# hsinnan75/MapCaller

Measured on AMD Instinct MI355X. Metric: reads/sec (150 bp PE vs GRCh38) at 1/2/4/8 MI355X; SAM CIGAR bit-exact, higher is better.
Workload: dtype u64/int32; 1 GPU; synthetic GRCh38-sized genome, 3100 Mbp (synthetic: GRCh38 is unavailable offline; repeat landscape in the detail record), 4000000 pairs x 150 bp PE per step per GPU (sub 0.005, ins 0.001, del 0.001 per base), -alg ksw2

## Files before the change

include/mcx.h:

```cpp
#ifndef MCX_H
#define MCX_H
#include <stdint.h>

#ifdef __cplusplus
extern "C" {
#endif

typedef struct mcx_index mcx_index;
typedef struct mcx_ctx mcx_ctx;

enum mcx_status {
    MCX_OK = 0,
    MCX_ERR_IO = -1,
    MCX_ERR_ARG = -2,
    MCX_ERR_DEVICE = -3,
    MCX_ERR_CAPACITY = -4,
    MCX_ERR_UNSUPPORTED = -5
};

const char *mcx_last_error(void);
int mcx_device_count(void);

#define MCX_INDEX_SAMPLED 0
#define MCX_INDEX_FULL 1
// ... 20 lines not shown
    int64_t max_batch_reads;
} mcx_opts;
void mcx_opts_default(mcx_opts *);

int mcx_ctx_create(const mcx_index *, const mcx_opts *, mcx_ctx **out);
typedef struct mcx_fit {
    int32_t pair_records_trimmed;
    int32_t batch_halvings;
    int32_t single_detail_set;
    int32_t pad;
    int64_t max_batch_reads;
    int64_t hbm_free_bytes;
    int64_t hbm_taken_bytes;
} mcx_fit;
int mcx_ctx_create_fit(mcx_index *, const mcx_opts *, int with_profile, int paired, int max_dup, int max_clip, mcx_ctx **out, uint32_t **planes, mcx_fit *fit);
void mcx_ctx_free(mcx_ctx *);

int mcx_bwt_search_batch(mcx_ctx *, const uint8_t *seqs, const uint32_t *seq_off, const int32_t *start, uint32_t n,
                         int32_t *len, int32_t *freq, uint64_t *loc);
int mcx_extend_batch(mcx_ctx *, int alg, const uint8_t *q, const uint32_t *q_off, const uint8_t *t,
                     const uint32_t *t_off, uint32_t n, uint8_t *ops, int32_t *ops_len, int32_t *score);
int mcx_extend_lanes(mcx_ctx *, int alg, int form, int strip, uint32_t blocks, const uint8_t *q, const uint32_t *q_off, const uint8_t *t,
                     const uint32_t *t_off, uint32_t n, uint8_t *ops, int32_t *ops_len, int32_t *score, void *summaries);

typedef struct mcx_aln {
    int64_t pos;
    int64_t mate_pos;
    int32_t chr;
    int32_t flag;
    int32_t mapq;
    int32_t tlen;
    int32_t nm, as, xs;
    int32_t n_cigar;
    int32_t fwd;
    int32_t has_mate;
    int32_t cigar_off;
    int32_t pad;
} mcx_aln;

typedef struct mcx_aln32 {
    uint32_t pos_lo, mate_lo;
    uint8_t pos_hi, mate_hi;
    uint8_t mapq;
    uint8_t bits;
    int32_t tlen;
    uint16_t flag;
// ... 140 lines not shown
```

mapcaller_amd/api.py:

```python
from __future__ import annotations

import ctypes as C
import os
from typing import List, Optional, Tuple

import numpy as np

_HERE = os.path.dirname(os.path.abspath(__file__))
LIB_PATH = os.environ.get("MCX_LIB") or os.path.join(_HERE, "libmcx.so")
CIGAR_STRIDE = 32
CIGAR_SLACK = 65536


def cigar_pool_words(n_reads):
    return n_reads * CIGAR_STRIDE + CIGAR_SLACK


def pack_reads(bases, lens=None):
    import torch
    n, rlen = bases.shape
    row_words = (rlen + 15) // 16
    lut = torch.zeros(256, dtype=torch.int64, device=bases.device)
    for i, ch in enumerate(b"ACGT"):
        lut[ch] = i
# ... 3 lines not shown
    b64 = bases.long()
    if lens is None:
        lens_t = torch.full((n,), rlen, dtype=torch.int64, device=bases.device)
    else:
        lens_t = lens.to(bases.device).long()
    inside = torch.arange(rlen, device=bases.device)[None, :] < lens_t[:, None]
    codes = lut[b64] * inside
    pad = row_words * 16 - rlen
    if pad:
        codes = torch.nn.functional.pad(codes, (0, pad))
    shifts = (30 - 2 * torch.arange(16, device=bases.device)).long()
    words = (codes.reshape(n, row_words, 16) << shifts).sum(-1)
    words = torch.where(words >= 2 ** 31, words - 2 ** 32, words).to(torch.int32)
    bad = (~known[b64]) & inside
    r, pos = torch.nonzero(bad, as_tuple=True)
    odd = (r << 32) | (pos << 8) | b64[r, pos]
    return (words.contiguous().cpu().pin_memory(), lens_t.to(torch.int32).cpu().pin_memory(), odd.cpu().pin_memory() if odd.numel() else torch.zeros(1, dtype=torch.int64).pin_memory(),
            int(odd.numel()), row_words)


SYMBOLS = [
    "mcx_last_error", "mcx_device_count", "mcx_pack_row", "mcx_host_cpus", "mcx_gz_inflate", "mcx_index_load", "mcx_index_build", "mcx_index_from_codes", "mcx_index_save", "mcx_index_free", "mcx_index_trim",
    "mcx_index_genome_size", "mcx_index_n_chr", "mcx_index_chr_name", "mcx_index_chr_len", "mcx_index_hbm_bytes",
    "mcx_opts_default", "mcx_ctx_create", "mcx_ctx_create_fit", "mcx_ctx_free", "mcx_bwt_search_batch", "mcx_extend_batch", "mcx_extend_lanes",
    "mcx_avg_init", "mcx_map_batch_dev", "mcx_map_batch", "mcx_cigar_words", "mcx_map_files", "mcx_map_files_ex", "mcx_file_opts_default",
    "mcx_profile_attach", "mcx_profile_settle", "mcx_profile_finalize", "mcx_profile_sparse", "mcx_planes_alloc", "mcx_planes_free", "mcx_planes_bytes",
    "mcx_vcf_defaults", "mcx_call_variants",
    "mcx_batch_begin", "mcx_batch_sums", "mcx_batch_replay", "mcx_batch_end", "mcx_avg_walk", "mcx_batch_totals", "mcx_batch_check", "mcx_avg_advance", "mcx_exchange_local", "mcx_exchange_local_free",
    "mcx_profile_sparse_shard", "mcx_batch_end_keys", "mcx_batch_accumulate",
    "mcx_stream_submit", "mcx_stream_submit_packed", "mcx_stream_map", "mcx_stream_collect", "mcx_stream_next", "mcx_stream_mapped",
    "mcx_stream_map32", "mcx_stream_mapped32",
    "mcx_ctx_set_multi", "mcx_multi_lines", "mcx_multi_copy", "mcx_stream_multi",
    "mcx_sam_format_dev", "mcx_sam_format", "mcx_sam_header",
]
COMM_LIB_PATH = os.path.join(_HERE, "libmcx_comm.so")
COMM_SYMBOLS = ["mcx_comm_init_all", "mcx_comm_unique_id", "mcx_comm_init_rank", "mcx_comm_free", "mcx_comm_rank", "mcx_comm_size",
                "mcx_profile_reduce", "mcx_comm_exchange", "mcx_comm_exchange_free"]


class McxError(RuntimeError):
    pass


class Opts(C.Structure):
    _fields_ = [("alg", C.c_int32), ("max_pos_diff", C.c_int32), ("max_mismatch_rate", C.c_float),
                ("max_read_len", C.c_int32), ("max_batch_reads", C.c_int64)]

# ... 184 lines not shown
    L.mcx_last_error.restype = C.c_char_p
    L.mcx_index_genome_size.restype = C.c_int64
    L.mcx_index_hbm_bytes.restype = C.c_int64
    L.mcx_index_chr_name.restype = C.c_char_p
    L.mcx_index_load.argtypes = [C.c_char_p, C.c_int, C.c_int, C.POINTER(C.c_void_p)]
    L.mcx_index_build.argtypes = [C.c_char_p, C.c_char_p, C.c_int]
    L.mcx_index_from_codes.argtypes = [C.c_void_p, C.c_int32, C.POINTER(C.c_int32), C.POINTER(C.c_char_p), C.c_int, C.c_int,
                                       C.POINTER(C.c_void_p), C.POINTER(C.c_double)]
    L.mcx_index_save.argtypes = [C.c_void_p, C.c_char_p]
    L.mcx_index_trim.argtypes = [C.c_void_p, C.c_int]
    for f in (L.mcx_index_free, L.mcx_ctx_free):
        f.argtypes = [C.c_void_p]
        f.restype = None
    for f in (L.mcx_index_genome_size, L.mcx_index_n_chr, L.mcx_index_hbm_bytes):
        f.argtypes = [C.c_void_p]
    L.mcx_index_chr_name.argtypes = [C.c_void_p, C.c_int32]
    L.mcx_index_chr_len.argtypes = [C.c_void_p, C.c_int32]
    L.mcx_opts_default.argtypes = [C.POINTER(Opts)]
    L.mcx_opts_default.restype = None
    L.mcx_ctx_create.argtypes = [C.c_void_p, C.POINTER(Opts), C.POINTER(C.c_void_p)]
    L.mcx_ctx_create_fit.argtypes = [C.c_void_p, C.POINTER(Opts), C.c_int, C.c_int, C.c_int, C.c_int, C.POINTER(C.c_void_p), C.POINTER(C.c_void_p), C.POINTER(Fit)]
    L.mcx_bwt_search_batch.argtypes = [C.c_void_p] + [C.c_void_p] * 3 + [C.c_uint32] + [C.c_void_p] * 3
    L.mcx_extend_batch.argtypes = [C.c_void_p, C.c_int] + [C.c_void_p] * 4 + [C.c_uint32] + [C.c_void_p] * 3
    L.mcx_extend_lanes.argtypes = [C.c_void_p, C.c_int, C.c_int, C.c_int, C.c_uint32] + [C.c_void_p] * 4 + [C.c_uint32] + [C.c_void_p] * 4
    L.mcx_avg_init.argtypes = [C.POINTER(C.c_int64)]
    L.mcx_avg_init.restype = None
    for f in (L.mcx_map_batch_dev, L.mcx_map_batch):
        f.argtypes = [C.c_void_p, C.c_void_p, C.c_void_p, C.c_uint32, C.c_int, C.POINTER(C.c_int64), C.c_void_p,
                      C.c_void_p, C.POINTER(Stats)]
    L.mcx_map_files.argtypes = [C.c_void_p, C.c_char_p, C.c_char_p, C.c_char_p, C.POINTER(Stats)]
    L.mcx_map_files_ex.argtypes = [C.c_void_p, C.c_char_p, C.c_char_p, C.POINTER(FileOpts), C.c_char_p, C.POINTER(Stats)]
    L.mcx_file_opts_default.argtypes = [C.POINTER(FileOpts)]
    L.mcx_file_opts_default.restype = None
    L.mcx_profile_attach.argtypes = [C.c_void_p, C.c_void_p, C.c_int, C.c_int]
    L.mcx_profile_settle.argtypes = [C.c_void_p]
    L.mcx_profile_finalize.argtypes = [C.c_void_p, C.c_void_p]
    L.mcx_profile_sparse.argtypes = [C.c_void_p, C.POINTER(C.POINTER(SparseRec)), C.POINTER(C.c_uint64)]
    L.mcx_profile_sparse_shard.argtypes = [C.c_void_p, C.POINTER(C.POINTER(SparseRec)), C.POINTER(C.c_uint64)]
    L.mcx_batch_begin.argtypes = [C.c_void_p, C.c_void_p, C.c_void_p, C.c_uint32, C.c_int, C.c_int32, C.c_int64, C.c_void_p, C.c_void_p, C.POINTER(Stats)]
    L.mcx_batch_sums.argtypes = [C.c_void_p, C.POINTER(C.c_uint32)] + [C.POINTER(C.POINTER(C.c_uint32))] * 3
    L.mcx_batch_replay.argtypes = [C.c_void_p, C.c_void_p, C.POINTER(C.c_uint32), C.POINTER(Stats)]
    L.mcx_batch_end.argtypes = [C.c_void_p, C.POINTER(Stats)]
    L.mcx_batch_end_keys.argtypes = [C.c_void_p, C.POINTER(Stats), C.POINTER(C.POINTER(C.c_uint64)), C.POINTER(C.c_uint64)]
    L.mcx_batch_accumulate.argtypes = [C.c_void_p, C.c_void_p, C.c_uint64, C.c_uint32, C.c_uint32]
    L.mcx_avg_walk.argtypes = [C.POINTER(C.c_int64), C.c_void_p, C.c_void_p, C.c_uint32, C.c_void_p]
    L.mcx_avg_walk.restype = None
# ... 394 lines not shown
        _check(lib().mcx_bwt_search_batch(self._h, buf.ctypes.data, off.ctypes.data, st.ctypes.data, n, ln.ctypes.data,
                                          fr.ctypes.data, loc.ctypes.data), "mcx_bwt_search_batch")
        return ln, fr, loc

    def extend(self, alg: str, qs: List[bytes], ts: List[bytes]):
        n = len(qs)
        qo = np.zeros(n + 1, dtype=np.uint32)
        to = np.zeros(n + 1, dtype=np.uint32)
        qo[1:] = np.cumsum([len(s) for s in qs])
        to[1:] = np.cumsum([len(s) for s in ts])
        qb = np.frombuffer(b"".join(qs), dtype=np.uint8).copy()
        tb = np.frombuffer(b"".join(ts), dtype=np.uint8).copy()
        ops = np.zeros(int(qo[-1]) + int(to[-1]) + 16, dtype=np.uint8)
        ol = np.zeros(n, dtype=np.int32)
        sc = np.zeros(n, dtype=np.int32)
        _check(lib().mcx_extend_batch(self._h, 0 if alg == "nw" else 1, qb.ctypes.data, qo.ctypes.data, tb.ctypes.data,
                                      to.ctypes.data, n, ops.ctypes.data, ol.ctypes.data, sc.ctypes.data), "mcx_extend_batch")
        out = []
        for i in range(n):
            b = int(qo[i]) + int(to[i])
            out.append(ops[b:b + int(ol[i])].tobytes().decode())
        return out, sc

    def extend_lanes(self, alg: str, form: int, strip: int, qs: List[bytes], ts: List[bytes], blocks: int = 0, summaries: bool = False):
        n = len(qs)
        qo = np.zeros(n + 1, dtype=np.uint32)
        to = np.zeros(n + 1, dtype=np.uint32)
        qo[1:] = np.cumsum([len(s) for s in qs])
        to[1:] = np.cumsum([len(s) for s in ts])
        qb = np.frombuffer(b"".join(qs) + b"\0", dtype=np.uint8).copy()
        tb = np.frombuffer(b"".join(ts) + b"\0", dtype=np.uint8).copy()
        ops = np.zeros(int(qo[-1]) + int(to[-1]) + 16, dtype=np.uint8)
        ol = np.zeros(n, dtype=np.int32)
        sc = np.zeros(n, dtype=np.int32)
        sm = np.zeros(n, dtype=DP_SUMMARY_DTYPE) if summaries else None
        _check(lib().mcx_extend_lanes(self._h, 0 if alg == "nw" else 1, form, strip, blocks, qb.ctypes.data, qo.ctypes.data, tb.ctypes.data,
                                      to.ctypes.data, n, ops.ctypes.data, ol.ctypes.data, sc.ctypes.data, sm.ctypes.data if summaries else None),
               "mcx_extend_lanes")
        out = []
        for i in range(n):
            b = int(qo[i]) + int(to[i])
            out.append(ops[b:b + int(ol[i])].tobytes().decode())
        return out, ol, sc, sm

    def close(self):
        if self._h:
# ... 85 lines not shown
```

mapcaller_amd/csrc/mcx_ctx.h:

```cpp
#ifndef MCX_CTX_H
#define MCX_CTX_H
#include <hip/hip_runtime.h>
#include <algorithm>
#include <atomic>
#include <chrono>
#include <cmath>
#include <cstdio>
#include <cstdlib>
#include <cstring>
#include <string>
#include <type_traits>
#include <vector>

#include "../../include/mcx.h"
#include "mcx_dp.h"
#include "mcx_dp_lane2.h"
#include "mcx_simple.h"
#include "mcx_profile.h"
#include "mcx_internal.h"

using namespace mcx;

#define HIP_TRY(expr)                                                                                  \
    do {                                                                                               \
// ... 170 lines not shown
            uint32_t *h_index = nullptr, *h_cig = nullptr; mcx_aln32 *h_recs = nullptr; uint32_t h_rec_cap = 0, h_word_cap = 0;
        } mx;
    } slot[3];
    const Slot *collected = nullptr;
    hipStream_t h2d_stream = nullptr, d2h_stream = nullptr;
    uint64_t stream_seq = 0, stream_bytes_in = 0, stream_bytes_out = 0;
    void *d_scan_tmp = nullptr; size_t scan_tmp_bytes = 0;
    void *files_state = nullptr; void (*files_drop)(void *) = nullptr;
    void *sam_state = nullptr; void (*sam_drop)(void *) = nullptr;
    uint8_t *d_bases = nullptr; uint32_t *d_off = nullptr; AlnRec *d_recs = nullptr; uint32_t *d_cig = nullptr;
    struct Multi {
        bool on = false, ready = false;
        uint32_t rec_cap = 0, word_cap = 0;
        AlnRec *d_pool = nullptr; uint32_t *d_pool_cig = nullptr; uint32_t *d_cnt = nullptr; uint4 *d_ref = nullptr;
        uint32_t *d_counts = nullptr;
        uint32_t *d_index = nullptr, *d_windex = nullptr;
        AlnRec *d_out = nullptr; uint32_t *d_out_cig = nullptr; uint32_t out_cap = 0, out_wcap = 0;
        void *d_tmp = nullptr; size_t tmp_bytes = 0;
        uint32_t n_reads = 0, n_recs = 0, n_words = 0;
    } mx;
};

int reserve_tier0(mcx_ctx *c, int paired, uint64_t n_reads);
void pack_reads(const ReadBatch &rb, int paired, int wpad, int tpr, uint32_t *out, uint32_t *any_n, uint8_t *odd_flag, hipStream_t s);
int launch_dp(const Knobs &kn, const PassRes &R, const Ctx &cx, const JobSinks &sinks, const ReadBatch &rb, const PairSel &sel, int rlen_max);
uint64_t lane_short_words(int which);
uint64_t lane_stride_words(bool nw, int rows, int strips);
int profile_keys(mcx_ctx *c);
int profile_queue(mcx_ctx *c);
int profile_collect(mcx_ctx *c);
int archive_append(mcx_ctx *c, mcx_ctx::Archive &a, const SparseRec *d_src, uint64_t n, hipStream_t on = nullptr);
int profile_foreign(mcx_ctx *c, const uint64_t *h_all, uint64_t n_all);
int sort_reserve(mcx_ctx *c, uint64_t n);
int profile_accumulate(mcx_ctx *c, const uint64_t *h_all, uint64_t n_all, uint32_t slot_stride, uint32_t own_slot);

#endif
```

mapcaller_amd/csrc/mcx_pipeline.hip:

```cpp
#include "mcx_ctx.h"
#include <hipcub/hipcub.hpp>

static thread_local std::string g_err;
static int fail(int code, const std::string &msg) { g_err = msg; return code; }
int mcx_set_error(int code, const std::string &msg) { return fail(code, msg); }
extern "C" const char *mcx_last_error(void) { return g_err.c_str(); }
extern "C" int mcx_device_count(void)
{
    int n = 0;
    if (hipGetDeviceCount(&n) != hipSuccess) return 0;
    return n;
}

struct EndsLds { int64_t pos[kLdsEnds]; int32_t chr[kLdsEnds]; };

static __device__ __forceinline__ void stage_ends(IndexView &ix, EndsLds &l)
{
    if (ix.n_ends <= kLdsEnds) {
        for (int i = threadIdx.x; i < ix.n_ends; i += blockDim.x) { l.pos[i] = ix.end_pos[i]; l.chr[i] = ix.end_chr[i]; }
        __syncthreads();
        ix.end_pos = l.pos; ix.end_chr = l.chr;
    }
}

// ... 4 lines not shown
        uint32_t r = pair * nr + s;
        rd[s].ascii = rb.bases + rb.off[r];
        rd[s].rlen = (int32_t)(rb.off[r + 1] - rb.off[r]);
        rd[s].flipped = (cx.pm.paired && s == 1) ? 1 : 0;
        rd[s].codes = (cx.packed && !(cx.read_ext[r] >> 31)) ? cx.packed + (uint64_t)r * cx.wpad : nullptr;
#ifdef MCX_DEBUG_NO_CODES
        rd[s].codes = nullptr;
#endif
    }
}

struct SeedOut {
    uint2 *tasks;
    uint32_t *n_tasks;
    uint32_t task_cap;
    uint32_t *read_ext;
    uint32_t *read_blocks;
    const uint32_t *packed;
    int wpad;
    uint32_t *queue;
    const uint8_t *src_state; Layout src_lay; Caps src_caps;
};

static __device__ __forceinline__ U4 load16_unaligned(const uint8_t *p)
{
    const uintptr_t a = (uintptr_t)p;
    const U4 *q = (const U4 *)(a & ~(uintptr_t)15);
    const U4 lo = q[0];
    const unsigned sh = (unsigned)(a & 15);
    if (sh == 0) return lo;
    const U4 hi = q[1];
    const unsigned qd = sh >> 2, b = sh & 3;
    uint32_t s0, s1, s2, s3, s4;
    switch (qd) {
    case 0: s0 = lo.x; s1 = lo.y; s2 = lo.z; s3 = lo.w; s4 = hi.x; break;
    case 1: s0 = lo.y; s1 = lo.z; s2 = lo.w; s3 = hi.x; s4 = hi.y; break;
    case 2: s0 = lo.z; s1 = lo.w; s2 = hi.x; s3 = hi.y; s4 = hi.z; break;
    default: s0 = lo.w; s1 = hi.x; s2 = hi.y; s3 = hi.z; s4 = hi.w; break;
    }
    U4 r;
    r.x = __builtin_amdgcn_alignbyte(s1, s0, b); r.y = __builtin_amdgcn_alignbyte(s2, s1, b);
    r.z = __builtin_amdgcn_alignbyte(s3, s2, b); r.w = __builtin_amdgcn_alignbyte(s4, s3, b);
    return r;
}

static __device__ __forceinline__ void pack4(uint32_t w, bool comp, uint32_t &codes, uint32_t &flags, uint32_t &lower)
{
    const uint32_t c = w & 0xDFDFDFDFu;
    auto zero_bytes = [](uint32_t t) { return ~(((t & 0x7F7F7F7Fu) + 0x7F7F7F7Fu) | t | 0x7F7F7F7Fu); };
    const uint32_t member = (zero_bytes(c ^ 0x41414141u) | zero_bytes(c ^ 0x43434343u) | zero_bytes(c ^ 0x47474747u) | zero_bytes(c ^ 0x54545454u)) >> 7;
    const uint32_t h = (c >> 1) & 0x03030303u;
    uint32_t code = h ^ ((h >> 1) & 0x01010101u);
    if (comp) code ^= 0x03030303u;
    code &= member * 3u;
    const uint32_t y = __builtin_bswap32(code), n = __builtin_bswap32(member ^ 0x01010101u);
    codes = (y | (y >> 6) | (y >> 12) | (y >> 18)) & 0xFFu;
    flags = (n | (n >> 7) | (n >> 14) | (n >> 21)) & 0xFu;
    const uint32_t l = __builtin_bswap32((w >> 5) & 0x01010101u);
    lower = (l | (l >> 7) | (l >> 14) | (l >> 21)) & 0xFu;
}

static __device__ __forceinline__ void pack16(const ReadRef &rd, int i0, uint32_t &codes, uint32_t &flags, uint32_t &odd)
{
    const int rlen = rd.rlen;
    int n = rlen - i0; if (n > 16) n = 16;
    codes = 0; flags = 0xFFFFu; odd = 0;
    if (n <= 0) return;
    const int a0 = rd.flipped ? rlen - i0 - n : i0;
    U4 v = load16_unaligned(rd.ascii + a0);
    if (rd.flipped) {
        const U4 t = v;
        v.x = __builtin_bswap32(t.w); v.y = __builtin_bswap32(t.z); v.z = __builtin_bswap32(t.y); v.w = __builtin_bswap32(t.x);
    }
    uint32_t c0, f0, c1, f1, c2, f2, c3, f3, l0, l1, l2, l3;
    pack4(v.x, rd.flipped != 0, c0, f0, l0); pack4(v.y, rd.flipped != 0, c1, f1, l1); pack4(v.z, rd.flipped != 0, c2, f2, l2); pack4(v.w, rd.flipped != 0, c3, f3, l3);
    uint32_t c = (c0 << 24) | (c1 << 16) | (c2 << 8) | c3, f = (f0 << 12) | (f1 << 8) | (f2 << 4) | f3, o = f | (l0 << 12) | (l1 << 8) | (l2 << 4) | l3;
    if (n < 16) {
        const int pad = 16 - n;
        if (rd.flipped) { c <<= 2 * pad; f = (f << pad) & 0xFFFFu; o = (o << pad) & 0xFFFFu; }
        else { c &= ~0u << (2 * pad); o &= ~0u << pad; }
        f |= (1u << pad) - 1u;
        if (!rd.flipped) f &= 0xFFFFu;
    }
    codes = c; flags = f; odd = o & 0xFFFFu;
}

__global__ void __launch_bounds__(256) k_pack_reads(ReadBatch rb, int paired, int wpad, int tpr, uint32_t *out, uint32_t *any_n, uint8_t *odd_flag)
{
    const uint64_t t = (uint64_t)blockIdx.x * blockDim.x + threadIdx.x;
    const uint32_t r = (uint32_t)(t / (uint32_t)tpr);
    const int m = (int)(t % (uint32_t)tpr);
    if (r >= rb.n_reads) return;
    ReadRef rd;
    rd.ascii = rb.bases + rb.off[r]; rd.rlen = (int)(rb.off[r + 1] - rb.off[r]); rd.flipped = (paired && (r & 1)) ? 1 : 0;
    const int rlen = rd.rlen, nc = (rlen + 15) >> 4, nmw = (rlen + 31) >> 5;
    if (nc + 1 + nmw + 1 > wpad) return;
    uint32_t *o = out + (uint64_t)r * wpad;
    if (m < nmw) {
        uint32_t c0, f0, c1, f1, o0, o1;
        pack16(rd, 32 * m, c0, f0, o0);
        pack16(rd, 32 * m + 16, c1, f1, o1);
        if (odd_flag && (o0 | o1)) atomicOr((uint32_t *)(odd_flag + (r & ~3u)), 2u << (8 * (r & 3)));
        o[2 * m] = c0;
        if (2 * m + 1 < nc) o[2 * m + 1] = c1;
        o[nc + 1 + m] = (f0 << 16) | f1;
        const int left = rlen - 32 * m;
        if (((f0 << 16) | f1) & (left >= 32 ? ~0u : ~(0xFFFFFFFFu >> left))) atomicOr(any_n, 1u);
    } else if (m == nmw) {
        o[nc] = 0u;
        o[nc + 1 + nmw] = 0xFFFFFFFFu;
    }
}

void pack_reads(const ReadBatch &rb, int paired, int wpad, int tpr, uint32_t *out, uint32_t *any_n, uint8_t *odd_flag, hipStream_t s)
{
    k_pack_reads<<<(unsigned)(((uint64_t)rb.n_reads * (uint64_t)tpr + 255) / 256), 256, 0, s>>>(rb, paired, wpad, tpr, out, any_n, odd_flag);
}

constexpr int kSeedReadsPerLane = 4;


static inline int seed_reads_per_lane(uint64_t n_reads) { return n_reads >= (uint64_t)1 << 21 ? kSeedReadsPerLane : (n_reads >= (uint64_t)1 << 19 ? 2 : 1); }

#ifndef MCX_SEED_WAVES
#define MCX_SEED_WAVES 1
#endif
#ifdef MCX_SEED_STATS
__device__ unsigned long long g_seed_hist[2][24];
#endif
__global__ void __launch_bounds__(256, MCX_SEED_WAVES) k_seed(Ctx cx, ReadBatch rb, PairSel sel, SeedOut so, int pk_words, int reads_per_lane, int fm_budget)
{
    extern __shared__ uint32_t pk_lds[];
    const int nr = cx.pm.paired ? 2 : 1;
    const uint32_t total = sel.n * nr;
    const int lane = threadIdx.x & 63;
    const uint64_t lt_mask = lane == 0 ? 0ull : (~0ull >> (64 - lane));
    const uint32_t chunk = 64u * (uint32_t)reads_per_lane;
    PackedRead pk; pk.w = pk_lds + threadIdx.x; pk.stride = blockDim.x; pk.n_code = 0;
    bool have = false;
// ... 1999 lines not shown
    if (int rc = reserve_tier0(c, paired, n_reads)) return rc;
    br.rb.bases = d_bases; br.rb.off = d_off; br.rb.n_reads = n_reads;
    br.paired = paired; br.read_base = read_base;
    br.recs = (AlnRec *)d_aln; br.cig = d_cigar; br.stats = stats;
    br.cig_cap = (uint32_t)std::min<uint64_t>((uint64_t)MCX_CIGAR_POOL_WORDS(n_reads), 0xFFFFFFFFu); br.cig_words = 0;
    br.n_pairs = paired ? n_reads / 2 : n_reads;
    br.n_chunks = (br.n_pairs + kReadChunkSize / 2 - 1) / (kReadChunkSize / 2);
    br.mapped = 0; br.sums_valid = false; br.d_ok = br.d_ds = nullptr;
    c->tail.queued = c->tail.ran = false;
    HIP_TRY(hipMemsetAsync(c->d_batch_flags, 0, 4 * sizeof(uint32_t), s));
    c->mx.ready = false;
    if (c->mx.on) HIP_TRY(hipMemsetAsync(c->mx.d_cnt, 0, 4 * sizeof(uint32_t), s));
    c->last_paired = paired ? 1 : 0;
    if (vouched) c->t0.h_cnt[1] = (uint32_t)c->rlen_max;
    else {
        k_max_read_len<<<512, 256, 0, s>>>(d_off, n_reads, c->d_batch_flags + 1);
        HIP_TRY(hipMemcpyAsync(c->t0.h_cnt, c->d_batch_flags, 4 * sizeof(uint32_t), hipMemcpyDeviceToHost, s));
        HIP_TRY(hipStreamSynchronize(s));
        if (c->t0.h_cnt[1] > (uint32_t)c->rlen_max)
            return fail(MCX_ERR_UNSUPPORTED, "a read of " + std::to_string(c->t0.h_cnt[1]) + " bases is longer than max_read_len (" + std::to_string(c->rlen_max) + ")");
    }
    {
        HIP_TRY(hipEventRecord(c->ev_pack[0], s));
        const int tpr = ((int)c->t0.h_cnt[1] + 31) / 32 + 1;
        br.longest = c->t0.h_cnt[1];
        if (c->prof_planes) HIP_TRY(hipMemsetAsync(c->d_admit, c->kn.prof_by_column ? 2 : 0, ((size_t)n_reads + 3) & ~(size_t)3, s));
        if (vouched && pre.packed && pre.bases == d_bases && pre.paired == (paired ? 1 : 0) && !c->prof_planes) {
            c->packed_now = pre.packed;
            HIP_TRY(hipMemcpyAsync(c->d_batch_flags + 3, pre.any_n, sizeof(uint32_t), hipMemcpyDeviceToDevice, s));
        } else {
            c->packed_now = c->d_packed;
            pack_reads(br.rb, paired, c->wpad, tpr, c->d_packed, c->d_batch_flags + 3, c->prof_planes ? c->d_admit : nullptr, s);
        }
        HIP_TRY(hipGetLastError());
        HIP_TRY(hipEventRecord(c->ev_pack[1], s));
    }
    c->later.kept_now = false;
    if (c->prof_planes && c->later.have && c->tail.want) {
        auto &L = c->later;
        L.kept_now = true;
        HIP_TRY(hipEventRecord(L.begun, s));
        HIP_TRY(hipStreamWaitEvent(L.keep_stream, L.begun, 0));
        k_keep_reads<<<2048, 256, 0, L.keep_stream>>>(d_bases, d_off, n_reads, L.d_keep_bases, L.d_keep_off);
        HIP_TRY(hipGetLastError());
        HIP_TRY(hipEventRecord(L.kept, L.keep_stream));
    }
    int rc;
    br.ms_setup = std::chrono::duration<double, std::milli>(std::chrono::steady_clock::now() - br.t0).count();
    rc = run_selection(c, br.rb, paired, nullptr, nullptr, est0, br.n_pairs, br.recs, d_cigar, stats, true);
    br.t_begun = std::chrono::steady_clock::now();
    if (rc) return rc;
    if (c->tail.queued) memcpy(c->t0.h_cnt + CNT_N, c->tail.h + 2, sizeof br.hs);
    else {
        unsigned long long *d_sum = (unsigned long long *)c->t0.d_cnt;
        HIP_TRY(hipMemsetAsync(c->t0.d_cnt, 0, CNT_N * sizeof(uint32_t), s));
// ... 488 lines not shown
                                    uint32_t n, int32_t *len, int32_t *freq, uint64_t *loc)
{
    if (!c || !seqs || !seq_off || !start || !len || !freq || !loc) return fail(MCX_ERR_ARG, "mcx_bwt_search_batch: null argument");
    if (n == 0) return 0;
    HIP_TRY(hipSetDevice(c->idx->device));
    uint8_t *d_seq = nullptr; uint32_t *d_off = nullptr; int32_t *d_start = nullptr, *d_len = nullptr, *d_freq = nullptr; uint64_t *d_loc = nullptr;
    int rc = 0;
    size_t nb = seq_off[n];
    if ((rc = dmalloc(&d_seq, nb + 16)) || (rc = dmalloc(&d_off, (size_t)n + 1)) || (rc = dmalloc(&d_start, n)) ||
        (rc = dmalloc(&d_len, n)) || (rc = dmalloc(&d_freq, n)) || (rc = dmalloc(&d_loc, (size_t)n * kOccThr))) return rc;
    HIP_TRY(hipMemcpy(d_seq, seqs, nb, hipMemcpyHostToDevice));
    HIP_TRY(hipMemcpy(d_off, seq_off, ((size_t)n + 1) * 4, hipMemcpyHostToDevice));
    HIP_TRY(hipMemcpy(d_start, start, (size_t)n * 4, hipMemcpyHostToDevice));
    k_bwt_search<<<(n + 255) / 256, 256, 0, c->t0.stream>>>(c->idx->view, d_seq, d_off, d_start, n, d_len, d_freq, d_loc);
    HIP_TRY(hipGetLastError());
    HIP_TRY(hipStreamSynchronize(c->t0.stream));
    HIP_TRY(hipMemcpy(len, d_len, (size_t)n * 4, hipMemcpyDeviceToHost));
    HIP_TRY(hipMemcpy(freq, d_freq, (size_t)n * 4, hipMemcpyDeviceToHost));
    HIP_TRY(hipMemcpy(loc, d_loc, (size_t)n * kOccThr * 8, hipMemcpyDeviceToHost));
    (void)hipFree(d_seq); (void)hipFree(d_off); (void)hipFree(d_start); (void)hipFree(d_len); (void)hipFree(d_freq); (void)hipFree(d_loc);
    return 0;
}

extern "C" int mcx_cigar_words(mcx_ctx *c, uint32_t *n_words)
{
    if (!c || !n_words) return fail(MCX_ERR_ARG, "mcx_cigar_words: null argument");
    *n_words = c->run.cig_words;
    return 0;
}

const mcx_index *mcx_ctx_index(const mcx_ctx *c) { return c->idx; }
int mcx_ctx_max_read_len(const mcx_ctx *c) { return c->rlen_max; }
bool mcx_ctx_has_profile(const mcx_ctx *c) { return c->prof_planes != nullptr; }
uint64_t mcx_ctx_max_reads(const mcx_ctx *c) { return c->max_reads; }
void **mcx_ctx_files_slot(mcx_ctx *c, void (*drop)(void *)) { c->files_drop = drop; return &c->files_state; }
void **mcx_ctx_sam_slot(mcx_ctx *c, void (*drop)(void *)) { c->sam_drop = drop; return &c->sam_state; }
void *mcx_ctx_stream(mcx_ctx *c) { return (void *)c->t0.stream; }
void *mcx_pinned_alloc(size_t bytes) { void *p = nullptr; return hipHostMalloc(&p, bytes ? bytes : 1, hipHostMallocDefault) == hipSuccess ? p : nullptr; }
void mcx_pinned_free(void *p) { if (p) (void)hipHostFree(p); }
```

mapcaller_amd/csrc/mcx_stream.hip:

```cpp
#include "mcx_ctx.h"
#include <hipcub/hipcub.hpp>

__global__ void __launch_bounds__(256) k_copy16(const U4 *__restrict__ src, U4 *__restrict__ dst, uint64_t n16)
{
    for (uint64_t i = (uint64_t)blockIdx.x * blockDim.x + threadIdx.x; i < n16; i += (uint64_t)gridDim.x * blockDim.x) dst[i] = src[i];
}

static int bulk_copy(mcx_ctx *c, void *dst, const void *src, size_t bytes, hipMemcpyKind kind, hipStream_t s)
{
    if (bytes == 0) return 0;
    static const char *mode = getenv("MCX_STREAM_KERNEL_COPY");
    static const int blocks = getenv("MCX_COPY_BLOCKS") ? atoi(getenv("MCX_COPY_BLOCKS")) : 512;
    const bool use_dma = mode == nullptr || (!strcmp(mode, "in") && kind != hipMemcpyHostToDevice) || (!strcmp(mode, "out") && kind != hipMemcpyDeviceToHost);
    const size_t n16 = bytes / 16;
    bool mapped = false;
    {
        hipPointerAttribute_t a;
        const void *host = kind == hipMemcpyHostToDevice ? src : dst;
        if (hipPointerGetAttributes(&a, host) == hipSuccess) mapped = a.type == hipMemoryTypeHost;
        else (void)hipGetLastError();
    }
    if (use_dma || !mapped || n16 == 0 || ((uintptr_t)dst & 15) || ((uintptr_t)src & 15)) { HIP_TRY(hipMemcpyAsync(dst, src, bytes, kind, s)); return 0; }
    k_copy16<<<blocks, 256, 0, s>>>((const U4 *)src, (U4 *)dst, (uint64_t)n16);
    HIP_TRY(hipGetLastError());
// ... 107 lines not shown
        HIP_TRY(hipMalloc(&c->d_scan_tmp, c->scan_tmp_bytes));
    }
    if ((rc = bulk_copy(c, sl->d_codes, codes, (size_t)n_reads * row_words * 4, hipMemcpyHostToDevice, s))) return rc;
    if ((rc = bulk_copy(c, sl->d_len, len, (size_t)n_reads * 4, hipMemcpyHostToDevice, s))) return rc;
    if (n_odd && (rc = bulk_copy(c, sl->d_odd, odd, (size_t)n_odd * 8, hipMemcpyHostToDevice, s))) return rc;
    HIP_TRY(hipMemsetAsync(sl->d_off, 0, 4, s));
    size_t tmp = c->scan_tmp_bytes;
    HIP_TRY(hipcub::DeviceScan::InclusiveSum(c->d_scan_tmp, tmp, sl->d_len, sl->d_off + 1, (int)n_reads, s));
    const uint64_t threads = (uint64_t)n_reads * row_words;
    HIP_TRY(hipMemsetAsync(sl->d_err, 0, 4, s));
    k_unpack_reads<<<(unsigned)((threads + 255) / 256), 256, 0, s>>>(sl->d_codes, row_words, sl->d_off, n_reads, sl->d_bases, c->max_bases,
                                                                   std::min<uint32_t>(row_words * 16u, (uint32_t)c->rlen_max), sl->d_err);
    if (n_odd) k_apply_odd<<<(n_odd + 255) / 256, 256, 0, s>>>(sl->d_odd, n_odd, sl->d_off, n_reads, sl->d_bases, c->max_bases);
    k_neutralize<<<256, 256, 0, s>>>(sl->d_off, n_reads, sl->d_err);
    HIP_TRY(hipGetLastError());
    sl->lens_checked = true;
    sl->prepacked = false;
    if (!c->prof_planes && !c->kn.no_prepack) {
        if (!sl->d_prepack) {
            if ((rc = dmalloc(&sl->d_prepack, c->max_reads * (uint64_t)c->wpad))) return rc;
            if ((rc = dmalloc(&sl->d_any_n, 1))) return rc;
        }
        ReadBatch rb; rb.bases = sl->d_bases; rb.off = sl->d_off; rb.n_reads = n_reads;
        const int tpr = (c->rlen_max + 31) / 32 + 1;
        HIP_TRY(hipMemsetAsync(sl->d_any_n, 0, 4, s));
        pack_reads(rb, c->last_paired, c->wpad, tpr, sl->d_prepack, sl->d_any_n, nullptr, s);
        HIP_TRY(hipGetLastError());
        sl->prepacked = true; sl->pre_paired = c->last_paired;
    }
    HIP_TRY(hipEventRecord(sl->in_ready, s));
    sl->n_reads = n_reads; sl->state = 1; sl->seq = ++c->stream_seq;
    c->stream_bytes_in += (uint64_t)n_reads * row_words * 4 + (uint64_t)n_reads * 4 + (uint64_t)n_odd * 8;
    return 0;
}

extern "C" int mcx_stream_submit(mcx_ctx *c, const uint8_t *bases, const uint32_t *off, uint32_t n_reads)
{
    if (!c || !bases || !off || n_reads == 0) return mcx_set_error(MCX_ERR_ARG, "mcx_stream_submit: bad argument");
    if (n_reads > c->max_reads) return mcx_set_error(MCX_ERR_ARG, "batch larger than max_batch_reads");
    if (off[n_reads] > c->max_bases) return mcx_set_error(MCX_ERR_ARG, "batch holds more bases than max_batch_reads * max_read_len");
    HIP_TRY(hipSetDevice(c->idx->device));
    mcx_ctx::Slot *sl = nullptr;
    int rc = stream_slot(c, &sl);
    if (rc) return rc;
    if (sl->d_err) HIP_TRY(hipMemsetAsync(sl->d_err, 0, 4, c->h2d_stream));
    sl->lens_checked = false; sl->prepacked = false;
    if ((rc = bulk_copy(c, sl->d_bases, bases, off[n_reads], hipMemcpyHostToDevice, c->h2d_stream))) return rc;
    if ((rc = bulk_copy(c, sl->d_off, off, (size_t)(n_reads + 1) * 4, hipMemcpyHostToDevice, c->h2d_stream))) return rc;
    HIP_TRY(hipEventRecord(sl->in_ready, c->h2d_stream));
// ... 190 lines not shown
```

Baseline: 533.0 million reads/s.

## Stage read bases and packed rows through LDS in the pack kernel

Rewrites k_pack_reads so each block handles a group of reads. The block copies their ASCII bases into LDS with coalesced 16-byte loads, packs 16-base chunks from LDS into an LDS row buffer, then writes whole rows to global memory coalesced. N/odd detection becomes per-block flags with one atomic each, instead of scattered unaligned global loads and per-thread atomics. The per-base pack arithmetic is also simplified. It adds a test entry point mcx_pack_reads_dev, and it risks LDS occupancy limits and edge cases when reads overflow the staging capacity.

```diff
diff --git a/include/mcx.h b/include/mcx.h
--- a/include/mcx.h
+++ b/include/mcx.h
@@ -66,6 +66,8 @@
                      const uint32_t *t_off, uint32_t n, uint8_t *ops, int32_t *ops_len, int32_t *score);
 int mcx_extend_lanes(mcx_ctx *, int alg, int form, int strip, uint32_t blocks, const uint8_t *q, const uint32_t *q_off, const uint8_t *t,
                      const uint32_t *t_off, uint32_t n, uint8_t *ops, int32_t *ops_len, int32_t *score, void *summaries);
+int mcx_pack_reads_dev(mcx_ctx *, const uint8_t *bases, const uint32_t *off, uint32_t n_reads, int paired, uint32_t *rows, uint32_t row_words,
+                       uint32_t extra, uint32_t *any_n, uint8_t *flags);
 
 typedef struct mcx_aln {
     int64_t pos;
diff --git a/mapcaller_amd/api.py b/mapcaller_amd/api.py
--- a/mapcaller_amd/api.py
+++ b/mapcaller_amd/api.py
@@ -49,7 +49,7 @@
 SYMBOLS = [
     "mcx_last_error", "mcx_device_count", "mcx_pack_row", "mcx_host_cpus", "mcx_gz_inflate", "mcx_index_load", "mcx_index_build", "mcx_index_from_codes", "mcx_index_save", "mcx_index_free", "mcx_index_trim",
     "mcx_index_genome_size", "mcx_index_n_chr", "mcx_index_chr_name", "mcx_index_chr_len", "mcx_index_hbm_bytes",
-    "mcx_opts_default", "mcx_ctx_create", "mcx_ctx_create_fit", "mcx_ctx_free", "mcx_bwt_search_batch", "mcx_extend_batch", "mcx_extend_lanes",
+    "mcx_opts_default", "mcx_ctx_create", "mcx_ctx_create_fit", "mcx_ctx_free", "mcx_bwt_search_batch", "mcx_extend_batch", "mcx_extend_lanes", "mcx_pack_reads_dev",
     "mcx_avg_init", "mcx_map_batch_dev", "mcx_map_batch", "mcx_cigar_words", "mcx_map_files", "mcx_map_files_ex", "mcx_file_opts_default",
     "mcx_profile_attach", "mcx_profile_settle", "mcx_profile_finalize", "mcx_profile_sparse", "mcx_planes_alloc", "mcx_planes_free", "mcx_planes_bytes",
     "mcx_vcf_defaults", "mcx_call_variants",
@@ -280,6 +280,7 @@
     L.mcx_ctx_create_fit.argtypes = [C.c_void_p, C.POINTER(Opts), C.c_int, C.c_int, C.c_int, C.c_int, C.POINTER(C.c_void_p), C.POINTER(C.c_void_p), C.POINTER(Fit)]
     L.mcx_bwt_search_batch.argtypes = [C.c_void_p] + [C.c_void_p] * 3 + [C.c_uint32] + [C.c_void_p] * 3
     L.mcx_extend_batch.argtypes = [C.c_void_p, C.c_int] + [C.c_void_p] * 4 + [C.c_uint32] + [C.c_void_p] * 3
+    L.mcx_pack_reads_dev.argtypes = [C.c_void_p, C.c_void_p, C.c_void_p, C.c_uint32, C.c_int, C.c_void_p, C.c_uint32, C.c_uint32, C.c_void_p, C.c_void_p]
     L.mcx_extend_lanes.argtypes = [C.c_void_p, C.c_int, C.c_int, C.c_int, C.c_uint32] + [C.c_void_p] * 4 + [C.c_uint32] + [C.c_void_p] * 4
     L.mcx_avg_init.argtypes = [C.POINTER(C.c_int64)]
     L.mcx_avg_init.restype = None
@@ -720,6 +721,18 @@
             out.append(ops[b:b + int(ol[i])].tobytes().decode())
         return out, sc
 
+    def pack_reads_dev(self, seqs: List[bytes], paired: bool, row_words: int, fill: int = 0, extra: int = 0):
+        n = len(seqs)
+        off = np.zeros(n + 1, dtype=np.uint32)
+        off[1:] = np.cumsum([len(s) for s in seqs])
+        buf = np.frombuffer(b"".join(seqs) + b"\0" * 16, dtype=np.uint8).copy()
+        rows = np.full(n * row_words + extra, fill, dtype=np.uint32)
+        any_n = C.c_uint32(0xFFFFFFFF)
+        flags = np.full(max(n, 1), 0xFF, dtype=np.uint8)
+        _check(lib().mcx_pack_reads_dev(self._h, buf.ctypes.data, off.ctypes.data, n, 1 if paired else 0, rows.ctypes.data, row_words, extra,
+                                        C.byref(any_n), flags.ctypes.data), "mcx_pack_reads_dev")
+        return rows, int(any_n.value), flags[:n]
+
     def extend_lanes(self, alg: str, form: int, strip: int, qs: List[bytes], ts: List[bytes], blocks: int = 0, summaries: bool = False):
         n = len(qs)
         qo = np.zeros(n + 1, dtype=np.uint32)
diff --git a/mapcaller_amd/csrc/mcx_ctx.h b/mapcaller_amd/csrc/mcx_ctx.h
--- a/mapcaller_amd/csrc/mcx_ctx.h
+++ b/mapcaller_amd/csrc/mcx_ctx.h
@@ -216,7 +216,7 @@
 };
 
 int reserve_tier0(mcx_ctx *c, int paired, uint64_t n_reads);
-void pack_reads(const ReadBatch &rb, int paired, int wpad, int tpr, uint32_t *out, uint32_t *any_n, uint8_t *odd_flag, hipStream_t s);
+void pack_reads(const ReadBatch &rb, int paired, int wpad, int longest, uint32_t *out, uint32_t *any_n, uint8_t *odd_flag, hipStream_t s);
 int launch_dp(const Knobs &kn, const PassRes &R, const Ctx &cx, const JobSinks &sinks, const ReadBatch &rb, const PairSel &sel, int rlen_max);
 uint64_t lane_short_words(int which);
 uint64_t lane_stride_words(bool nw, int rows, int strips);
diff --git a/mapcaller_amd/csrc/mcx_pipeline.hip b/mapcaller_amd/csrc/mcx_pipeline.hip
--- a/mapcaller_amd/csrc/mcx_pipeline.hip
+++ b/mapcaller_amd/csrc/mcx_pipeline.hip
@@ -50,99 +50,129 @@
     const uint8_t *src_state; Layout src_lay; Caps src_caps;
 };
 
-static __device__ __forceinline__ U4 load16_unaligned(const uint8_t *p)
-{
-    const uintptr_t a = (uintptr_t)p;
-    const U4 *q = (const U4 *)(a & ~(uintptr_t)15);
-    const U4 lo = q[0];
-    const unsigned sh = (unsigned)(a & 15);
-    if (sh == 0) return lo;
-    const U4 hi = q[1];
-    const unsigned qd = sh >> 2, b = sh & 3;
-    uint32_t s0, s1, s2, s3, s4;
-    switch (qd) {
-    case 0: s0 = lo.x; s1 = lo.y; s2 = lo.z; s3 = lo.w; s4 = hi.x; break;
-    case 1: s0 = lo.y; s1 = lo.z; s2 = lo.w; s3 = hi.x; s4 = hi.y; break;
-    case 2: s0 = lo.z; s1 = lo.w; s2 = hi.x; s3 = hi.y; s4 = hi.z; break;
-    default: s0 = lo.w; s1 = hi.x; s2 = hi.y; s3 = hi.z; s4 = hi.w; break;
-    }
-    U4 r;
-    r.x = __builtin_amdgcn_alignbyte(s1, s0, b); r.y = __builtin_amdgcn_alignbyte(s2, s1, b);
-    r.z = __builtin_amdgcn_alignbyte(s3, s2, b); r.w = __builtin_amdgcn_alignbyte(s4, s3, b);
-    return r;
-}
-
-static __device__ __forceinline__ void pack4(uint32_t w, bool comp, uint32_t &codes, uint32_t &flags, uint32_t &lower)
+static __device__ __forceinline__ void lds_load16(const uint8_t *lds, int a, uint32_t v[4])
+{
+    const uint32_t *q = (const uint32_t *)(lds + (a & ~3));
+    const uint32_t b = (uint32_t)a & 3u, s0 = q[0], s1 = q[1], s2 = q[2], s3 = q[3], s4 = q[4];
+    v[0] = __builtin_amdgcn_alignbyte(s1, s0, b); v[1] = __builtin_amdgcn_alignbyte(s2, s1, b);
+    v[2] = __builtin_amdgcn_alignbyte(s3, s2, b); v[3] = __builtin_amdgcn_alignbyte(s4, s3, b);
+}
+
+static __device__ __forceinline__ void pack4(uint32_t w, uint32_t comp3, uint32_t &codes, uint32_t &flags, uint32_t &n_acc, uint32_t &odd_acc)
 {
     const uint32_t c = w & 0xDFDFDFDFu;
-    auto zero_bytes = [](uint32_t t) { return ~(((t & 0x7F7F7F7Fu) + 0x7F7F7F7Fu) | t | 0x7F7F7F7Fu); };
-    const uint32_t member = (zero_bytes(c ^ 0x41414141u) | zero_bytes(c ^ 0x43434343u) | zero_bytes(c ^ 0x47474747u) | zero_bytes(c ^ 0x54545454u)) >> 7;
+    const uint32_t is_t = ((c & ~(c << 1)) >> 2) & 0x01010101u;
+    const uint32_t t = (c & 0xF9F9F9F9u) ^ 0x41414141u ^ (is_t | (is_t << 4));
+    const uint32_t nm = ((((t & 0x7F7F7F7Fu) + 0x7F7F7F7Fu) | t) >> 7) & 0x01010101u;
     const uint32_t h = (c >> 1) & 0x03030303u;
-    uint32_t code = h ^ ((h >> 1) & 0x01010101u);
-    if (comp) code ^= 0x03030303u;
-    code &= member * 3u;
-    const uint32_t y = __builtin_bswap32(code), n = __builtin_bswap32(member ^ 0x01010101u);
-    codes = (y | (y >> 6) | (y >> 12) | (y >> 18)) & 0xFFu;
-    flags = (n | (n >> 7) | (n >> 14) | (n >> 21)) & 0xFu;
-    const uint32_t l = __builtin_bswap32((w >> 5) & 0x01010101u);
-    lower = (l | (l >> 7) | (l >> 14) | (l >> 21)) & 0xFu;
-}
-
-static __device__ __forceinline__ void pack16(const ReadRef &rd, int i0, uint32_t &codes, uint32_t &flags, uint32_t &odd)
-{
-    const int rlen = rd.rlen;
-    int n = rlen - i0; if (n > 16) n = 16;
-    codes = 0; flags = 0xFFFFu; odd = 0;
-    if (n <= 0) return;
-    const int a0 = rd.flipped ? rlen - i0 - n : i0;
-    U4 v = load16_unaligned(rd.ascii + a0);
-    if (rd.flipped) {
-        const U4 t = v;
-        v.x = __builtin_bswap32(t.w); v.y = __builtin_bswap32(t.z); v.z = __builtin_bswap32(t.y); v.w = __builtin_bswap32(t.x);
-    }
-    uint32_t c0, f0, c1, f1, c2, f2, c3, f3, l0, l1, l2, l3;
-    pack4(v.x, rd.flipped != 0, c0, f0, l0); pack4(v.y, rd.flipped != 0, c1, f1, l1); pack4(v.z, rd.flipped != 0, c2, f2, l2); pack4(v.w, rd.flipped != 0, c3, f3, l3);
-    uint32_t c = (c0 << 24) | (c1 << 16) | (c2 << 8) | c3, f = (f0 << 12) | (f1 << 8) | (f2 << 4) | f3, o = f | (l0 << 12) | (l1 << 8) | (l2 << 4) | l3;
+    const uint32_t code = (h ^ ((h >> 1) & 0x01010101u) ^ comp3) & ~(nm | (nm << 1));
+    uint32_t y = (code << 2) | (code >> 8);
+    y = (y << 4) | (y >> 16);
+    codes = y & 0xFFu;
+    uint32_t z = (nm << 1) | (nm >> 8);
+    z = (z << 2) | (z >> 16);
+    flags = z & 0xFu;
+    n_acc |= nm; odd_acc |= nm | ((w >> 5) & 0x01010101u);
+}
+
+static __device__ __forceinline__ void pack16(const uint8_t *lds, int a, bool flipped, int n, uint32_t &codes, uint32_t &flags, uint32_t &any_n, uint32_t &any_odd)
+{
+    uint32_t v[4];
+    lds_load16(lds, a, v);
+    if (flipped) {
+        const uint32_t t0 = v[0], t1 = v[1];
+        v[0] = __builtin_bswap32(v[3]); v[1] = __builtin_bswap32(v[2]); v[2] = __builtin_bswap32(t1); v[3] = __builtin_bswap32(t0);
+    }
     if (n < 16) {
-        const int pad = 16 - n;
-        if (rd.flipped) { c <<= 2 * pad; f = (f << pad) & 0xFFFFu; o = (o << pad) & 0xFFFFu; }
-        else { c &= ~0u << (2 * pad); o &= ~0u << pad; }
+        const int k = n < 0 ? 0 : n;
+        const uint64_t lo = k >= 8 ? ~0ull : ~(~0ull << (8 * k)), hi = k <= 8 ? 0ull : ~(~0ull << (8 * (k - 8)));
+        const uint32_t m[4] = {(uint32_t)lo, (uint32_t)(lo >> 32), (uint32_t)hi, (uint32_t)(hi >> 32)};
+        for (int d = 0; d < 4; d++) v[d] = (v[d] & m[d]) | (0x41414141u & ~m[d]);
+    }
+    const uint32_t comp3 = flipped ? 0x03030303u : 0u;
+    uint32_t c0, f0, c1, f1, c2, f2, c3, f3, na = 0, oa = 0;
+    pack4(v[0], comp3, c0, f0, na, oa); pack4(v[1], comp3, c1, f1, na, oa); pack4(v[2], comp3, c2, f2, na, oa); pack4(v[3], comp3, c3, f3, na, oa);
+    uint32_t c = (c0 << 24) | (c1 << 16) | (c2 << 8) | c3, f = (f0 << 12) | (f1 << 8) | (f2 << 4) | f3;
+    if (n < 16) {
+        const int pad = n < 0 ? 16 : 16 - n;
+        c = pad >= 16 ? 0u : (c >> (2 * pad)) << (2 * pad);
         f |= (1u << pad) - 1u;
-        if (!rd.flipped) f &= 0xFFFFu;
-    }
-    codes = c; flags = f; odd = o & 0xFFFFu;
-}
-
-__global__ void __launch_bounds__(256) k_pack_reads(ReadBatch rb, int paired, int wpad, int tpr, uint32_t *out, uint32_t *any_n, uint8_t *odd_flag)
-{
-    const uint64_t t = (uint64_t)blockIdx.x * blockDim.x + threadIdx.x;
-    const uint32_t r = (uint32_t)(t / (uint32_t)tpr);
-    const int m = (int)(t % (uint32_t)tpr);
-    if (r >= rb.n_reads) return;
-    ReadRef rd;
-    rd.ascii = rb.bases + rb.off[r]; rd.rlen = (int)(rb.off[r + 1] - rb.off[r]); rd.flipped = (paired && (r & 1)) ? 1 : 0;
-    const int rlen = rd.rlen, nc = (rlen + 15) >> 4, nmw = (rlen + 31) >> 5;
-    if (nc + 1 + nmw + 1 > wpad) return;
-    uint32_t *o = out + (uint64_t)r * wpad;
-    if (m < nmw) {
-        uint32_t c0, f0, c1, f1, o0, o1;
-        pack16(rd, 32 * m, c0, f0, o0);
-        pack16(rd, 32 * m + 16, c1, f1, o1);
-        if (odd_flag && (o0 | o1)) atomicOr((uint32_t *)(odd_flag + (r & ~3u)), 2u << (8 * (r & 3)));
-        o[2 * m] = c0;
-        if (2 * m + 1 < nc) o[2 * m + 1] = c1;
-        o[nc + 1 + m] = (f0 << 16) | f1;
-        const int left = rlen - 32 * m;
-        if (((f0 << 16) | f1) & (left >= 32 ? ~0u : ~(0xFFFFFFFFu >> left))) atomicOr(any_n, 1u);
-    } else if (m == nmw) {
-        o[nc] = 0u;
-        o[nc + 1 + nmw] = 0xFFFFFFFFu;
-    }
-}
-
-void pack_reads(const ReadBatch &rb, int paired, int wpad, int tpr, uint32_t *out, uint32_t *any_n, uint8_t *odd_flag, hipStream_t s)
-{
-    k_pack_reads<<<(unsigned)(((uint64_t)rb.n_reads * (uint64_t)tpr + 255) / 256), 256, 0, s>>>(rb, paired, wpad, tpr, out, any_n, odd_flag);
+    }
+    codes = c; flags = f; any_n = na; any_odd = oa;
+}
+
+constexpr uint32_t kPackSlack = 48;
+__global__ void __launch_bounds__(256) k_pack_reads(ReadBatch rb, int paired, int wpad, int rpb_log2, uint32_t cap, uint32_t step_q, uint32_t step_r,
+                                                    uint32_t *out, uint32_t *any_n, uint8_t *odd_flag)
+{
+    extern __shared__ U4 pack_lds[];
+    const uint32_t tid = threadIdx.x, rpb = 1u << rpb_log2, tpr = 256u >> rpb_log2;
+    uint8_t *asc = (uint8_t *)pack_lds + kPackSlack;
+    uint32_t *rows = (uint32_t *)(asc + cap + kPackSlack);
+    uint32_t *offs = rows + rpb * (uint32_t)wpad, *used = offs + rpb + 1, *odd = used + rpb, *any = odd + rpb;
+    const uint32_t r0 = blockIdx.x << rpb_log2, nrd = min(rpb, rb.n_reads - r0);
+    if (tid <= nrd) offs[tid] = rb.off[r0 + tid];
+    if (tid < rpb) { used[tid] = 0u; odd[tid] = 0u; }
+    if (tid == 0) *any = 0u;
+    __syncthreads();
+    const uint32_t li = tid >> (8 - rpb_log2), j0 = tid & (tpr - 1u);
+    const uint32_t base = offs[0] & ~15u;
+    {
+        const uint32_t n16 = min((offs[nrd] - base + 15u) >> 4, cap >> 4);
+        const U4 *src = (const U4 *)(rb.bases + base);
+        for (uint32_t i = tid; i < n16; i += 256u) ((U4 *)asc)[i] = src[i];
+    }
+    __syncthreads();
+    if (li < nrd) {
+        const uint32_t o0 = offs[li], o1 = offs[li + 1];
+        const int rlen = (int)(o1 - o0), nc = (rlen + 15) >> 4, nmw = (rlen + 31) >> 5;
+        if (o0 >= base && o1 >= o0 && o1 - base <= cap && nc + 1 + nmw + 1 <= wpad) {
+            const bool flipped = paired && ((r0 + li) & 1u);
+            uint32_t *row = rows + li * (uint32_t)wpad;
+            uint32_t an = 0, ao = 0;
+            for (int j = (int)j0; j <= 2 * nmw; j += (int)tpr) {
+                if (j == 2 * nmw) { row[nc] = 0u; row[nc + 1 + nmw] = 0xFFFFFFFFu; used[li] = (uint32_t)(nc + 1 + nmw + 1); break; }
+                const int i0 = 16 * j;
+                uint32_t c, f, a, o;
+                pack16(asc, (int)(o0 - base) + (flipped ? rlen - i0 - 16 : i0), flipped, rlen - i0, c, f, a, o);
+                if (j < nc) row[j] = c;
+                ((uint16_t *)(row + nc + 1 + (j >> 1)))[(j & 1) ^ 1] = (uint16_t)f;
+                an |= a; ao |= o;
+            }
+            if (an) *any = 1u;
+            if (ao) odd[li] = 1u;
+        }
+    }
+    __syncthreads();
+    {
+        uint32_t *to = out + (uint64_t)r0 * (uint32_t)wpad;
+        const uint32_t total = nrd * (uint32_t)wpad;
+        uint32_t rl = tid / (uint32_t)wpad, k = tid - rl * (uint32_t)wpad;
+        for (uint32_t i = tid; i < total; i += 256u) {
+            if (k < used[rl]) to[i] = rows[i];
+            rl += step_q; k += step_r;
+            if (k >= (uint32_t)wpad) { k -= (uint32_t)wpad; rl++; }
+        }
+    }
+    if (tid < nrd && odd_flag && odd[tid]) { const uint32_t r = r0 + tid; atomicOr((uint32_t *)(odd_flag + (r & ~3u)), 2u << (8 * (r & 3u))); }
+    if (tid == 0 && *any) atomicOr(any_n, 1u);
+}
+
+void pack_reads(const ReadBatch &rb, int paired, int wpad, int longest, uint32_t *out, uint32_t *any_n, uint8_t *odd_flag, hipStream_t s)
+{
+    int fit = 32 * wpad / 3;
+    while (packed_words(fit + 1) <= wpad) fit++;
+    while (fit > 0 && packed_words(fit) > wpad) fit--;
+    const uint32_t len = (uint32_t)std::max(1, std::min(longest, fit));
+    auto lds_bytes = [&](int lg, uint32_t &cap) {
+        cap = ((len << lg) + 15u + 15u) & ~15u;
+        return (size_t)cap + 2 * kPackSlack + ((size_t)wpad << lg) * 4 + (3 * ((size_t)1 << lg) + 2) * 4;
+    };
+    int lg = 6;
+    uint32_t cap = 0;
+    while (lg > 0 && lds_bytes(lg, cap) > 32768) lg--;
+    const size_t lds = lds_bytes(lg, cap);
+    k_pack_reads<<<(unsigned)(((uint64_t)rb.n_reads + (1u << lg) - 1) >> lg), 256, lds, s>>>(rb, paired, wpad, lg, cap, 256u / (uint32_t)wpad, 256u % (uint32_t)wpad, out, any_n, odd_flag);
 }
 
 constexpr int kSeedReadsPerLane = 4;
@@ -2188,7 +2218,6 @@
     }
     {
         HIP_TRY(hipEventRecord(c->ev_pack[0], s));
-        const int tpr = ((int)c->t0.h_cnt[1] + 31) / 32 + 1;
         br.longest = c->t0.h_cnt[1];
         if (c->prof_planes) HIP_TRY(hipMemsetAsync(c->d_admit, c->kn.prof_by_column ? 2 : 0, ((size_t)n_reads + 3) & ~(size_t)3, s));
         if (vouched && pre.packed && pre.bases == d_bases && pre.paired == (paired ? 1 : 0) && !c->prof_planes) {
@@ -2196,7 +2225,7 @@
             HIP_TRY(hipMemcpyAsync(c->d_batch_flags + 3, pre.any_n, sizeof(uint32_t), hipMemcpyDeviceToDevice, s));
         } else {
             c->packed_now = c->d_packed;
-            pack_reads(br.rb, paired, c->wpad, tpr, c->d_packed, c->d_batch_flags + 3, c->prof_planes ? c->d_admit : nullptr, s);
+            pack_reads(br.rb, paired, c->wpad, (int)c->t0.h_cnt[1] , c->d_packed, c->d_batch_flags + 3, c->prof_planes ? c->d_admit : nullptr, s);
         }
         HIP_TRY(hipGetLastError());
         HIP_TRY(hipEventRecord(c->ev_pack[1], s));
@@ -2731,6 +2760,42 @@
     return 0;
 }
 
+extern "C" int mcx_pack_reads_dev(mcx_ctx *c, const uint8_t *bases, const uint32_t *off, uint32_t n_reads, int paired, uint32_t *rows, uint32_t row_words,
+                                  uint32_t extra, uint32_t *any_n, uint8_t *flags)
+{
+    if (!c || !bases || !off || !rows || !any_n || !flags) return fail(MCX_ERR_ARG, "mcx_pack_reads_dev: null argument");
+    if (row_words != (uint32_t)c->wpad) return fail(MCX_ERR_ARG, "mcx_pack_reads_dev: row_words is " + std::to_string(row_words) + ", the context's rows have " + std::to_string(c->wpad) + " words");
+    *any_n = 0;
+    if (n_reads == 0) return 0;
+    uint32_t longest = 0;
+    for (uint32_t r = 0; r < n_reads; r++) {
+        if (off[r + 1] < off[r]) return fail(MCX_ERR_ARG, "mcx_pack_reads_dev: offsets must not decrease");
+        longest = std::max(longest, off[r + 1] - off[r]);
+    }
+    if (longest > (uint32_t)c->rlen_max) return fail(MCX_ERR_UNSUPPORTED, "a read of " + std::to_string(longest) + " bases is longer than max_read_len (" + std::to_string(c->rlen_max) + ")");
+    HIP_TRY(hipSetDevice(c->idx->device));
+    uint8_t *d_bases = nullptr, *d_flags = nullptr; uint32_t *d_off = nullptr, *d_rows = nullptr, *d_any = nullptr;
+    const size_t nb = off[n_reads], n_words = (size_t)n_reads * row_words + extra, n_flags = ((size_t)n_reads + 3) & ~(size_t)3;
+    auto drop = [&]() { (void)hipFree(d_bases); (void)hipFree(d_flags); (void)hipFree(d_off); (void)hipFree(d_rows); (void)hipFree(d_any); };
+    int rc = 0;
+    if ((rc = dmalloc(&d_bases, nb + 16)) || (rc = dmalloc(&d_off, (size_t)n_reads + 1)) || (rc = dmalloc(&d_rows, n_words)) || (rc = dmalloc(&d_any, 1)) ||
+        (rc = dmalloc(&d_flags, n_flags))) { drop(); return rc; }
+    hipStream_t s = c->t0.stream;
+    hipError_t e = hipMemcpyAsync(d_bases, bases, nb, hipMemcpyHostToDevice, s);
+    if (e == hipSuccess) e = hipMemcpyAsync(d_off, off, ((size_t)n_reads + 1) * 4, hipMemcpyHostToDevice, s);
+    if (e == hipSuccess) e = hipMemcpyAsync(d_rows, rows, n_words * 4, hipMemcpyHostToDevice, s);
+    if (e == hipSuccess) e = hipMemsetAsync(d_any, 0, 4, s);
+    if (e == hipSuccess) e = hipMemsetAsync(d_flags, 0, n_flags, s);
+    if (e == hipSuccess) { pack_reads(ReadBatch{d_bases, d_off, n_reads}, paired ? 1 : 0, c->wpad, (int)longest, d_rows, d_any, d_flags, s); e = hipGetLastError(); }
+    if (e == hipSuccess) e = hipMemcpyAsync(rows, d_rows, n_words * 4, hipMemcpyDeviceToHost, s);
+    if (e == hipSuccess) e = hipMemcpyAsync(any_n, d_any, 4, hipMemcpyDeviceToHost, s);
+    if (e == hipSuccess) e = hipMemcpyAsync(flags, d_flags, n_reads, hipMemcpyDeviceToHost, s);
+    if (e == hipSuccess) e = hipStreamSynchronize(s);
+    drop();
+    if (e != hipSuccess) return fail(MCX_ERR_DEVICE, std::string("mcx_pack_reads_dev: ") + hipGetErrorString(e));
+    return 0;
+}
+
 extern "C" int mcx_cigar_words(mcx_ctx *c, uint32_t *n_words)
 {
     if (!c || !n_words) return fail(MCX_ERR_ARG, "mcx_cigar_words: null argument");
diff --git a/mapcaller_amd/csrc/mcx_stream.hip b/mapcaller_amd/csrc/mcx_stream.hip
--- a/mapcaller_amd/csrc/mcx_stream.hip
+++ b/mapcaller_amd/csrc/mcx_stream.hip
@@ -153,9 +153,8 @@
             if ((rc = dmalloc(&sl->d_any_n, 1))) return rc;
         }
         ReadBatch rb; rb.bases = sl->d_bases; rb.off = sl->d_off; rb.n_reads = n_reads;
-        const int tpr = (c->rlen_max + 31) / 32 + 1;
         HIP_TRY(hipMemsetAsync(sl->d_any_n, 0, 4, s));
-        pack_reads(rb, c->last_paired, c->wpad, tpr, sl->d_prepack, sl->d_any_n, nullptr, s);
+        pack_reads(rb, c->last_paired, c->wpad, c->rlen_max, sl->d_prepack, sl->d_any_n, nullptr, s);
         HIP_TRY(hipGetLastError());
         sl->prepacked = true; sl->pre_paired = c->last_paired;
     }
```

Measured after the change: 538.1 million reads/s (median of 6 runs). Within noise of the previous version (+1.0%).
